# gavrissh/training-operator

Hardware: AMD Instinct MI355X
Metric: job×node fit evals/sec + gang placements/sec, 1M-node inventory, 1/2/4/8 GPUs (higher is better)
Workload: dtype int64

## Files before the change

training-operator_amd/csrc/pe_kernels.h:

```cpp
#pragma once
#include <hip/hip_runtime.h>
#include <stdint.h>

namespace pe {

constexpr int D = 4;
constexpr uint64_t SCORE_MAX = (1ull << 40) - 1;
constexpr uint64_t NO_KEY = ~0ull;
constexpr int64_t NEVER = INT64_MIN;

struct alignas(64) ReqRec {
  int64_t q[D];
  uint32_t need;
  uint32_t pad_[7];
};
static_assert(sizeof(ReqRec) == 64, "ReqRec must be 64 B");

struct alignas(32) ReqRec32 {
  int32_t q[D];
  uint32_t need;
  uint32_t pad_[3];
};
static_assert(sizeof(ReqRec32) == 32, "ReqRec32 must be 32 B");

struct CandHdr {
  int32_t n;
  int32_t flags;
  uint64_t limit;
};
static_assert(sizeof(CandHdr) == 16, "CandHdr must be 16 B");
constexpr int32_t CAND_TIMEOUT = -1;
constexpr int32_t CAND_CORRUPT = -2;

__host__ __device__ inline size_t cand_group_bytes(int K) { return sizeof(CandHdr) + (size_t)K * sizeof(uint64_t); }

constexpr int FM_CH = 4;
constexpr int FM_JT = 256;
constexpr int SC_M = 16;
constexpr int SC_GT = 4;
constexpr int SC_SPAN = 64 * SC_M;
constexpr int SC_WPB = 16;
constexpr int MG_CAP = 16384;
constexpr int MG_THREADS = 1024;
constexpr int MG_SEL = 1024;

constexpr int AGG_SEG_JOBS = 256;
constexpr int64_t AGG_SEG_BYTES = 48 * 1024;
struct AggSegHdr {
  int64_t j0;
  int32_t nj, ng, nc;
  int32_t g0, c0;
  int32_t narrow;
};
static_assert(sizeof(AggSegHdr) == 32, "AggSegHdr must be 32 B");
__host__ __device__ inline int64_t agg_r16(int64_t x) { return (x + 15) & ~int64_t(15); }
struct AggKeys {
  int nd = 4;
  int fb = 1;
};
constexpr int AGG_MAX_KEYS = 16;
__host__ __device__ inline int64_t agg_req_bytes(int64_t nc, int nd, bool narrow) {
  return narrow ? 16 + agg_r16(nc * 4 * nd) : nc * 8 * nd;
}
__host__ __device__ inline void agg_seg_layout(int64_t nj, int64_t ng, int64_t nc, bool v1, int64_t off[7],
                                               AggKeys ak = AggKeys{}, bool narrow = false) {
  off[0] = (int64_t)sizeof(AggSegHdr);
  off[1] = off[0] + agg_r16((nj + 1) * 4);
  off[2] = off[1] + (v1 ? agg_r16(nj * 4) : 0);
  off[3] = off[2] + agg_r16(ng * 4);
  off[4] = off[3] + agg_r16((ng + 1) * 4);
  off[5] = off[4] + agg_req_bytes(nc, ak.nd, narrow);
  off[6] = off[5] + agg_r16(nc * ak.fb);
}
__host__ __device__ inline void agg_out_layout(int64_t J, int64_t off[4], AggKeys ak = AggKeys{}) {
  off[0] = 0;
  off[1] = agg_r16(J * 8 * ak.nd);
  off[2] = off[1] + agg_r16(J * 4);
  off[3] = off[2] + agg_r16(J * (ak.fb == 1 ? 1 : 2));
}

hipError_t launch_pg_agg_segments(hipStream_t s, int mode, const uint8_t* blob, const int64_t* seg_off, int64_t nseg,
                                  int64_t nbytes0, uint8_t* out, int64_t J, uint32_t* flag, uint32_t flag_val,
                                  uint32_t* done_ctr, AggKeys ak = AggKeys{});
constexpr int64_t AGG_KARG_BYTES = 512;
struct AggKarg {
  alignas(16) uint8_t b[AGG_KARG_BYTES];
};
hipError_t launch_pg_agg_karg(hipStream_t s, int mode, const AggKarg& blob, int64_t nbytes, uint8_t* out, int64_t J,
                              uint32_t* flag, uint32_t flag_val, AggKeys ak = AggKeys{});
hipError_t launch_pg_min_resources(hipStream_t s, int mode, int64_t n_jobs, const int32_t* job_group_off,
                                   const int32_t* min_member, const int32_t* group_replicas,
                                   const int32_t* group_cont_off, const int64_t* cont_req,
                                   const uint8_t* cont_flags, int64_t* out_res, uint8_t* out_present,
                                   int32_t* out_members, uint8_t* out_overflow);
hipError_t launch_pg_agg_wide(hipStream_t s, int mode, int64_t n_jobs, int n_keys, const int32_t* job_group_off,
                              const int32_t* min_member, const int32_t* group_replicas,
                              const int32_t* group_cont_off, const uint64_t* req_lo, const uint64_t* req_hi,
                              const uint32_t* cont_flags, uint64_t* out_lo, int64_t* out_hi, uint8_t* out_flag);

__host__ __device__ inline int64_t fm_word_index(int64_t j, int64_t c, int64_t Wt) {
  return ((j >> 4) * Wt + (c >> 2)) * 64 + (j & 15) * 4 + (c & 3);
}
hipError_t launch_fit_mask(hipStream_t s, const int64_t* res, int64_t stride, const uint32_t* labels,
                           int64_t Ns, int64_t Wt, const ReqRec* jobs, int64_t J, int64_t tiles_per_wave,
                           uint64_t* mask, unsigned long long* counts);

hipError_t launch_compress_res(hipStream_t s, const int64_t* res, int32_t* res32, int64_t stride, int64_t Ns,
                               const int* shift);
hipError_t launch_fit_mask32(hipStream_t s, const int32_t* res32, int64_t stride, const uint32_t* labels,
                             int64_t Ns, int64_t Wt, const ReqRec32* jobs, int64_t J, int64_t tiles_per_wave,
                             uint64_t* mask, unsigned long long* counts);

constexpr int CODE_FIELDS = 5;
constexpr int CODE_MAXV = 128;
struct CodeSpec {
  int off[CODE_FIELDS];
  int width[CODE_FIELDS];
  int nvals[CODE_FIELDS];
  uint32_t guard;
  int therm;
};
constexpr int FC_CH = 16;
constexpr int FC_JT = 64;

hipError_t launch_encode_nodes(hipStream_t s, const int64_t* res, int64_t stride, const uint32_t* labels, int64_t Ns,
                               int64_t n_pad, CodeSpec spec, const int64_t* vals, const uint32_t* needs, uint32_t* X);
hipError_t launch_fit_mask_coded(hipStream_t s, int therm, const uint32_t* X, int64_t Ns, int64_t node_stride,
                                 const uint32_t* jcode, uint32_t not_guard, int64_t J, int64_t tiles_per_wave,
                                 uint64_t* mask, unsigned long long* counts);

constexpr int PL_MAX = 32;
constexpr int PL_R = 4;
constexpr int PL_BLK = 64 * PL_R * 32;
struct PlaneSpec {
  int32_t n;
  int32_t kind[PL_MAX];
  int64_t val[PL_MAX];
};
hipError_t launch_encode_planes(hipStream_t s, const int64_t* res, int64_t stride, const uint32_t* labels,
                                int64_t Ns, int64_t nblk, const PlaneSpec& spec, const PlaneSpec* spec_d,
                                uint32_t* planes, unsigned long long* zero = nullptr,
                                int64_t n_zero = 0);
hipError_t launch_fit_mask_planes(hipStream_t s, const uint32_t* planes, int64_t nblk, const uint64_t* jcode,
                                  int64_t J, int64_t jobs_per_wave, uint32_t* mask, unsigned long long* counts);
hipError_t launch_fit_mask_planes_rows(hipStream_t s, const uint32_t* planes, int64_t nblk, const uint64_t* jcode,
                                       int64_t J, int64_t R, uint32_t* mask, unsigned long long* counts,
                                       int64_t pitch_blk, unsigned long long* unit_ctr = nullptr);
hipError_t launch_encode_planes_sets(hipStream_t s, const int64_t* res, int64_t stride, const uint32_t* labels,
                                     int64_t Ns, int64_t nblk, const PlaneSpec* specs, int nsets, uint32_t* planes);
hipError_t launch_fit_mask_planes_sets(hipStream_t s, const uint32_t* planes, int64_t nblk, const uint64_t* jcode,
                                       const int64_t* meta, int nsets, int64_t R, uint32_t* mask,
                                       unsigned long long* counts, int64_t pitch_blk);

constexpr int LD_MAXF = 4;
constexpr int LD_MAXL = 4;
constexpr int LD_MAXNEED = 64;
constexpr int LD_CODE = 16;
constexpr int LD_NEED_SLOT = 15;
__host__ __device__ constexpr int lds_field_off(int fi, int n4, int n3, int n2) {
  return fi <= n4                ? 4 * fi
         : fi <= n4 + n3         ? 4 * n4 + 3 * (fi - n4)
         : fi <= n4 + n3 + n2    ? 4 * n4 + 3 * n3 + 2 * (fi - n4 - n3)
                                 : 4 * n4 + 3 * n3 + 2 * n2 + (fi - n4 - n3 - n2);
}
__host__ __device__ constexpr int lds_need_slot(int n4, int n3, int n2, int n1) {
  return 4 * n4 + 3 * n3 + 2 * n2 + n1;
}
constexpr int LD_THREADS = 1024;
struct LdsSpec {
  int32_t nf;
  int32_t dim[LD_MAXF];
  int32_t L[LD_MAXF];
  uint32_t div[LD_MAXF][LD_MAXL];
  uint32_t mod[LD_MAXF][LD_MAXL];
  int32_t pbase[LD_MAXF][LD_MAXL];
  int32_t vlo[LD_MAXF][LD_MAXL];
  int32_t nv[LD_MAXF][LD_MAXL];
  int32_t nneed, need_pbase, nplanes, nfold;
  int32_t nx, xprod;
  int32_t xstride[LD_MAXF];
  uint32_t needs[LD_MAXNEED];
  int32_t fold_dim[D];
  int64_t fold_val[D];
  int64_t voff[LD_MAXF];
  int64_t m[LD_MAXF];
};
hipError_t launch_node_ranks(hipStream_t s, const int64_t* res, int64_t stride, const uint32_t* labels, int64_t Ns,
                             int64_t npad, const LdsSpec* spec, const int64_t* vals, uint32_t* ranks, uint32_t* aux);
hipError_t launch_fit_mask_lds(hipStream_t s, int W, const int shape[4], const LdsSpec* spec, int nplanes,
                               const uint32_t* ranks, int64_t npad, const uint32_t* aux, int64_t nblk,
                               const uint16_t* codes, int64_t J, int64_t R, int64_t Tpad, int64_t pitch_bytes,
                               uint8_t* mask, uint32_t* slots, uint32_t* units = nullptr);
hipError_t launch_lds_counts(hipStream_t s, const uint32_t* slots, const uint32_t* rows, int64_t nslots,
                             unsigned long long* counts);

hipError_t launch_prep_nodes(hipStream_t s, const int64_t* res, int64_t stride, int64_t Ns, uint64_t id_base,
                             uint64_t* kn, uint32_t* lo );
hipError_t launch_scan(hipStream_t s, const int64_t* res, int64_t stride, const uint32_t* labels, const uint64_t* kn,
                       const uint32_t* lo, int64_t Ns, uint64_t id_base, const ReqRec* groups, int Wg, uint64_t* cand,
                       int32_t* cnt, uint64_t* bound, int nwaves);

hipError_t launch_merge(hipStream_t s, const uint64_t* cand, const int32_t* cnt, const uint64_t* bound,
                        int nwaves, int K, uint8_t* out, int Wg);

constexpr int WK_ROUND = 1024;
constexpr int WK_MAXR = 16384;
constexpr uint64_t WK_INVALID = ~0ull;
#ifndef WK_MULTI
#define WK_MULTI 2
#endif
#ifndef WK_MULTI_AFTER
#define WK_MULTI_AFTER 1
#endif
struct WalkIndex {
  uint64_t* sk;
  int64_t* sr;
  uint32_t* sl;
  uint32_t* pos;
  uint64_t* rmin;
  int64_t* rmax;
  uint32_t* ror;
  int32_t* ovl;
  int32_t* ovl_n;
  uint32_t* in_ovl;
  uint32_t* ovl_idx;
  int64_t* ovl_res;
  uint32_t* ovl_lab;
  uint64_t* ovl_kn;
  unsigned long long* stat;
  int64_t sstride, nr;
};
hipError_t launch_walk_prep(hipStream_t s, const int64_t* res, int64_t stride, int64_t Ns, const uint64_t* kn,
                            const uint32_t* labels, uint64_t* kin, const WalkIndex& w, uint32_t* slow = nullptr);
hipError_t launch_walk_switch(hipStream_t s, const int64_t* res, int64_t stride, const uint32_t* labels, int64_t Ns,
                              const uint32_t* slow, const WalkIndex& nx);
hipError_t sort_keys_u64(void* temp, size_t* temp_bytes, const uint64_t* in, uint64_t* out, int64_t n, hipStream_t s);
hipError_t launch_walk_build(hipStream_t s, const int64_t* res, int64_t stride, const uint32_t* labels, int64_t Ns,
                             uint64_t id_base, const WalkIndex& w);
hipError_t launch_merge_shards(hipStream_t s, const uint8_t* gath, int world, int Wg, int K, uint8_t* out, uint32_t gen,
                               int64_t rank_stride = 0, const uint64_t* xstatus = nullptr, bool sys_scope = true);
constexpr int XW_THREADS = 256;
hipError_t launch_xwait(hipStream_t s, const uint8_t* gath, int world, int Wg, int K, int64_t rank_stride,
                        uint32_t in_gen, int64_t timeout_ticks, uint64_t* xstatus);
constexpr int RM_THREADS = 256, RM_MAX_WORLD = 16;
constexpr size_t RM_MAX_LDS = 64 * 1024;
size_t merge_ranked_lds(int world, int K);
hipError_t launch_merge_ranked(hipStream_t s, const uint8_t* gath, int world, int Wg, int K, uint8_t* out, uint32_t gen,
                               int64_t rank_stride = 0, const uint64_t* xstatus = nullptr, bool sys_scope = true);
hipError_t launch_empty_groups(hipStream_t s, int Wg, int K, uint8_t* out, uint32_t gen);
hipError_t launch_stall(hipStream_t s, int64_t ticks);
hipError_t launch_walk(hipStream_t s, const ReqRec* groups, int Wg, int K, const WalkIndex& w, const int64_t* res,
                       int64_t stride, const uint32_t* labels, int64_t Ns, uint64_t id_base, uint8_t* out,
                       uint32_t gen = 0, int K_stride = 0);

hipError_t launch_apply(hipStream_t s, int64_t* res, int64_t stride, const int64_t* upd, int64_t n, uint64_t id_base,
                        uint64_t* kn, uint32_t* lo, const uint32_t* labels, const WalkIndex* w,
                        const WalkIndex* nx = nullptr);

struct NodeUpd {
  int64_t local;
  int64_t res[D];
  uint32_t labels;
  int32_t island;
};
static_assert(sizeof(NodeUpd) == 48, "NodeUpd must be 48 B");
hipError_t launch_scatter_nodes(hipStream_t s, int64_t* res, int64_t* res0, int64_t stride, uint32_t* labels,
                                int32_t* island, const NodeUpd* upd, int64_t n);

constexpr int CP_THREADS = 256;
constexpr int CP_NPT = 4;
constexpr int CP_SPAN = CP_THREADS * CP_NPT;
constexpr int CP_TS = 64;
constexpr uint64_t CP_CAP_MAX = 2147483647;
__host__ __device__ inline int64_t cap_node_blocks(int64_t Ns) { return (Ns + CP_SPAN - 1) / CP_SPAN; }
struct alignas(32) CapShape {
  int64_t q[D];
  uint64_t m[D];
  uint32_t sh[D];
  uint32_t need;
  uint32_t pad_[3];
};
static_assert(sizeof(CapShape) == 96, "CapShape must be 96 B");
struct CapAcc {
  uint64_t slots;
  uint32_t max_node;
  uint32_t nodes;
};
static_assert(sizeof(CapAcc) == 16, "CapAcc must be 16 B");
hipError_t launch_gang_capacity(hipStream_t s, const int64_t* res, int64_t stride, const uint32_t* labels, int64_t Ns,
                                const CapShape* shapes, int64_t S, CapAcc* partials, CapAcc* out);

constexpr int DM_MAX_DOMAINS = 65536;
struct DomPick {
  uint32_t shape;
  int32_t count;
};
struct DomSel {
  uint64_t slots;
  int32_t domain;
  uint32_t feasible;
};
static_assert(sizeof(DomPick) == 8 && sizeof(DomSel) == 16, "DomPick / DomSel layout");
hipError_t launch_gang_capacity_domains(hipStream_t s, const int64_t* res, int64_t stride, const uint32_t* labels,
                                        const int32_t* island, int64_t Ns, const CapShape* shapes, int64_t S,
                                        int n_domains, uint64_t* dom_slots, uint32_t* dom_nodes);
hipError_t launch_domain_select(hipStream_t s, const uint64_t* dom_slots, int64_t s0, int64_t S, int n_domains,
                                const DomPick* picks, int64_t P, DomSel* out);

constexpr int TR_MAX_LEVELS = 4;
struct TreePick {
  uint32_t shape;
  int32_t count;
  int32_t max_level;
  int32_t pad_;
};
struct TreeSel {
  uint64_t slots;
  int32_t domain;
  int32_t level;
};
static_assert(sizeof(TreePick) == 16 && sizeof(TreeSel) == 16, "TreePick / TreeSel layout");
struct TreeLevels {
  int32_t n_levels;
  int32_t size[TR_MAX_LEVELS];
  int32_t col[TR_MAX_LEVELS];
  int32_t pitch;
};
hipError_t launch_tree_rollup(hipStream_t s, const uint64_t* lo_slots, const uint32_t* lo_nodes, int64_t lo_pitch,
                              const int32_t* start, const int32_t* child, int n_parents, int width, int64_t S,
                              uint64_t* up_slots, uint32_t* up_nodes, int64_t up_pitch);
hipError_t launch_tree_select(hipStream_t s, const uint64_t* leaf_slots, const uint64_t* upper_slots, int64_t s0,
                              int64_t S, const TreeLevels& levels, const TreePick* picks, int64_t P, TreeSel* out,
                              uint32_t* feasible);

}
```

training-operator_amd/csrc/pe_kernels.hip:

```cpp
#include <type_traits>

#include "pe_kernels.h"
#include "pe_wave.h"

namespace pe {

__device__ __forceinline__ uint64_t umin64(uint64_t a, uint64_t b) { return a < b ? a : b; }

__device__ __forceinline__ uint64_t wave_min_u64(uint64_t v) {
#pragma unroll
  for (int off = 32; off >= 1; off >>= 1) v = umin64(v, __shfl_xor(v, off, 64));
  return v;
}


__device__ __forceinline__ bool add_ovf(int64_t a, int64_t b, int64_t* r) { return __builtin_add_overflow(a, b, r); }
__device__ __forceinline__ bool mul_ovf(int64_t a, int64_t b, int64_t* r) { return __builtin_mul_overflow(a, b, r); }

template <int ND>
struct AggJob {
  int64_t acc[ND];
  uint32_t pres, members;
  int32_t pod_cnt;
  bool ovf;
// ... 1912 lines not shown
  if (tid < world) cnt[tid] = lds_lower_bound(lk + tid * K, hn[tid], L);
  __syncthreads();
  const int c = (K + 1 + world - 1) / world;
  int T = 0, have = 0;
  uint64_t U = 0;
  for (int r = 0; r < world; ++r) {
    const int hd = min(cnt[r], c);
    T += cnt[r];
    have += hd;
    if (hd > 0) U = umax64(U, lk[r * K + hd - 1]);
  }
  if (tid < world)
    mc[tid] = have >= K + 1 ? lds_lower_bound(lk + tid * K, cnt[tid], U + 1) : cnt[tid];
  __syncthreads();
  int M = 0, mx = 0, mq[RM_MAX_WORLD];
#pragma unroll
  for (int q = 0; q < RM_MAX_WORLD; ++q) {
    mq[q] = q < world ? mc[q] : 0;
    M += mq[q];
    mx = max(mx, mq[q]);
  }
  int top = 1;
  while (top * 2 <= mx) top *= 2;
  uint64_t* ok = lk + (size_t)world * K;
  for (int t = tid; t < M; t += RM_THREADS) {
    int r = 0, idx = t;
    while (idx >= mc[r]) {
      idx -= mc[r];
      ++r;
    }
    const uint64_t k = lk[r * K + idx];
    int pos[RM_MAX_WORLD];
#pragma unroll
    for (int q = 0; q < RM_MAX_WORLD; ++q) pos[q] = 0;
    for (int st = top; st > 0; st >>= 1) {
#pragma unroll
      for (int q = 0; q < RM_MAX_WORLD; ++q) {
        const int p = pos[q] + st;
        if (q < world && q != r && p <= mq[q] && lk[q * K + p - 1] < k) pos[q] = p;
      }
    }
    int rank = idx;
#pragma unroll
    for (int q = 0; q < RM_MAX_WORLD; ++q) rank += pos[q];
    if (rank <= K) ok[rank] = k;
  }
  __syncthreads();
  const int nout = T < K ? T : K;
  uint64_t* dst = reinterpret_cast<uint64_t*>(og + sizeof(CandHdr));
  for (int i = tid; i < nout; i += RM_THREADS) dst[i] = ok[i];
  if (tid == 0) {
    hp->n = nout;
    hp->limit = T > K ? ok[K] : L;
    if (gen == 0) hp->flags = 0;
  }
  asm volatile("s_waitcnt vmcnt(0)" ::: "memory");
  __syncthreads();
  if (tid == 0 && gen != 0) __hip_atomic_store(&hp->flags, (int32_t)gen, __ATOMIC_RELEASE, __HIP_MEMORY_SCOPE_SYSTEM);
}

size_t merge_ranked_lds(int world, int K) { return ((size_t)world * K + K + 1) * sizeof(uint64_t); }

hipError_t launch_merge_ranked(hipStream_t s, const uint8_t* gath, int world, int Wg, int K, uint8_t* out, uint32_t gen,
                               int64_t rank_stride, const uint64_t* xstatus, bool sys_scope) {
  if (Wg <= 0) return hipSuccess;
  if (world < 1 || world > RM_MAX_WORLD || K < 1 || merge_ranked_lds(world, K) > RM_MAX_LDS) return hipErrorInvalidValue;
  if (sys_scope)
    hipLaunchKernelGGL(merge_ranked_kernel<true>, dim3(Wg), dim3(RM_THREADS), merge_ranked_lds(world, K), s, gath, world,
                       Wg, K, out, gen, rank_stride, xstatus);
  else
    hipLaunchKernelGGL(merge_ranked_kernel<false>, dim3(Wg), dim3(RM_THREADS), merge_ranked_lds(world, K), s, gath, world,
                       Wg, K, out, gen, rank_stride, xstatus);
  return hipGetLastError();
}

__global__ __launch_bounds__(64) void empty_groups_kernel(int Wg, int K, uint8_t* __restrict__ out, uint32_t gen) {
  write_group(nullptr, 0, 0, NO_KEY, K, blockIdx.x, out, gen);
}

__global__ __launch_bounds__(64) void stall_kernel(int64_t ticks) {
  const long long t0 = wall_clock64();
  while (wall_clock64() - t0 < ticks) __builtin_amdgcn_s_sleep(127);
}

hipError_t launch_stall(hipStream_t s, int64_t ticks) {
  if (ticks <= 0 || ticks > (int64_t)30 * 100000000) return hipErrorInvalidValue;
  hipLaunchKernelGGL(stall_kernel, dim3(1), dim3(64), 0, s, ticks);
  return hipGetLastError();
}

hipError_t launch_empty_groups(hipStream_t s, int Wg, int K, uint8_t* out, uint32_t gen) {
  if (Wg <= 0) return hipSuccess;
  hipLaunchKernelGGL(empty_groups_kernel, dim3(Wg), dim3(64), 0, s, Wg, K, out, gen);
  return hipGetLastError();
}

hipError_t launch_merge(hipStream_t s, const uint64_t* cand, const int32_t* cnt, const uint64_t* bound, int nwaves,
                        int K, uint8_t* out, int Wg) {
  if (Wg <= 0) return hipSuccess;
  hipLaunchKernelGGL(merge_kernel, dim3(Wg), dim3(MG_THREADS), 0, s, cand, cnt, bound, nwaves, K, out);
  return hipGetLastError();
}


__device__ __forceinline__ void overlay_add(const WalkIndex& w, int64_t n, const int64_t (&r)[D], uint32_t lab,
                                            uint64_t Kn) {
  const int32_t i = atomicAdd(w.ovl_n, 1);
  w.ovl[i] = (int32_t)n;
  w.ovl_idx[n] = (uint32_t)i;
#pragma unroll
  for (int d = 0; d < D; ++d) w.ovl_res[d * w.sstride + i] = r[d];
  w.ovl_lab[i] = lab;
  w.ovl_kn[i] = Kn;
}

__global__ __launch_bounds__(256) void walk_prep_kernel(const int64_t* __restrict__ res, int64_t stride, int64_t Ns,
                                                        const uint64_t* __restrict__ kn,
                                                        const uint32_t* __restrict__ labels, uint64_t* __restrict__ kin,
                                                        WalkIndex w, uint32_t* __restrict__ slow) {
  const int64_t n = (int64_t)blockIdx.x * blockDim.x + threadIdx.x;
  if (n >= Ns) return;
  const int64_t r[D] = {res[n], res[stride + n], res[2 * stride + n], res[3 * stride + n]};
  const bool neg = (r[0] | r[1] | r[2] | r[3]) < 0;
  const uint64_t K = kn[n];
  uint64_t k = K;
  if (neg) {
    k = WK_INVALID;
  } else if (K == KEY_SLOW) {
    k = WK_INVALID;
    if (slow) {
      slow[n] = 1u;
    } else {
      w.in_ovl[n] = 1u;
      overlay_add(w, n, r, labels[n], KEY_SLOW);
    }
  }
  kin[n] = k;
}

hipError_t launch_walk_prep(hipStream_t s, const int64_t* res, int64_t stride, int64_t Ns, const uint64_t* kn,
                            const uint32_t* labels, uint64_t* kin, const WalkIndex& w, uint32_t* slow) {
  if (Ns <= 0) return hipSuccess;
  hipLaunchKernelGGL(walk_prep_kernel, dim3((unsigned)((Ns + 255) / 256)), dim3(256), 0, s, res, stride, Ns, kn, labels,
                     kin, w, slow);
  return hipGetLastError();
}

__global__ __launch_bounds__(256) void walk_switch_kernel(const int64_t* __restrict__ res, int64_t stride,
                                                          const uint32_t* __restrict__ labels, int64_t Ns,
                                                          const uint32_t* __restrict__ slow, WalkIndex nx) {
  const int64_t n = (int64_t)blockIdx.x * blockDim.x + threadIdx.x;
  if (n >= Ns) return;
  if (nx.in_ovl[n]) {
    const uint32_t p = nx.pos[n];
    if (p != ~0u) {
      nx.sk[p] = WK_INVALID;
      nx.pos[n] = ~0u;
    }
  } else if (slow[n]) {
    const int64_t r[D] = {res[n], res[stride + n], res[2 * stride + n], res[3 * stride + n]};
    nx.in_ovl[n] = 1u;
    overlay_add(nx, n, r, labels[n], KEY_SLOW);
  }
}

hipError_t launch_walk_switch(hipStream_t s, const int64_t* res, int64_t stride, const uint32_t* labels, int64_t Ns,
                              const uint32_t* slow, const WalkIndex& nx) {
  if (Ns <= 0) return hipSuccess;
  hipLaunchKernelGGL(walk_switch_kernel, dim3((unsigned)((Ns + 255) / 256)), dim3(256), 0, s, res, stride, labels, Ns,
                     slow, nx);
  return hipGetLastError();
}

__global__ __launch_bounds__(WK_ROUND) void walk_build_kernel(const int64_t* __restrict__ res, int64_t stride,
                                                              const uint32_t* __restrict__ labels, int64_t Ns,
                                                              uint64_t id_base, WalkIndex w) {
  __shared__ int64_t mx[D][WK_ROUND / 64];
  __shared__ uint32_t orl[WK_ROUND / 64];
  const int tid = threadIdx.x, lane = tid & 63, wave = tid >> 6;
  const int64_t r = blockIdx.x;
  const int64_t i = r * WK_ROUND + tid;
  const uint64_t K = i < Ns ? w.sk[i] : WK_INVALID;
  int64_t v[D] = {INT64_MIN, INT64_MIN, INT64_MIN, INT64_MIN};
  uint32_t lab = 0;
  if (K != WK_INVALID) {
    const int64_t n = (int64_t)((K & 0xFFFFFFull) - id_base);
    w.pos[n] = (uint32_t)i;
#pragma unroll
    for (int d = 0; d < D; ++d) {
      v[d] = res[d * stride + n];
      w.sr[d * w.sstride + i] = v[d];
    }
    lab = labels[n];
    w.sl[i] = lab;
  }
#pragma unroll
  for (int d = 0; d < D; ++d)
    for (int off = 32; off >= 1; off >>= 1) {
      const int64_t o = __shfl_xor(v[d], off, 64);
      v[d] = o > v[d] ? o : v[d];
    }
  for (int off = 32; off >= 1; off >>= 1) lab |= __shfl_xor(lab, off, 64);
  if (lane == 0) {
#pragma unroll
    for (int d = 0; d < D; ++d) mx[d][wave] = v[d];
    orl[wave] = lab;
  }
  __syncthreads();
  if (tid < D) {
    int64_t m = INT64_MIN;
    for (int k = 0; k < WK_ROUND / 64; ++k) m = mx[tid][k] > m ? mx[tid][k] : m;
    w.rmax[tid * w.nr + r] = m;
  } else if (tid == D) {
    uint32_t o = 0;
    for (int k = 0; k < WK_ROUND / 64; ++k) o |= orl[k];
    w.ror[r] = o;
    w.rmin[r] = w.sk[r * WK_ROUND];
  }
}

hipError_t launch_walk_build(hipStream_t s, const int64_t* res, int64_t stride, const uint32_t* labels, int64_t Ns,
                             uint64_t id_base, const WalkIndex& w) {
  if (Ns <= 0) return hipSuccess;
  hipLaunchKernelGGL(walk_build_kernel, dim3((unsigned)w.nr), dim3(WK_ROUND), 0, s, res, stride, labels, Ns, id_base,
                     w);
  return hipGetLastError();
}

__device__ __forceinline__ void step_append(TopkShared& s, int T0, int* cnt, uint64_t k, bool take) {
  const uint64_t bal = __ballot(take);
  if (bal == 0) return;
  const int rank = __builtin_amdgcn_mbcnt_hi((uint32_t)(bal >> 32), __builtin_amdgcn_mbcnt_lo((uint32_t)bal, 0));
  int base = 0;
  if (take && rank == 0) base = atomicAdd(cnt, __popcll(bal));
  base = T0 + __shfl(base, __ffsll((unsigned long long)bal) - 1, 64);
  if (take && base + rank < MG_CAP) s.keys[base + rank] = k;
}

#ifdef PE_WALK_PROF
__device__ unsigned long long walk_prof[32];
#define WPT(i) unsigned long long wpt##i = wall_clock64()
#else
#define WPT(i)
#endif

__global__ __launch_bounds__(WK_ROUND) void walk_kernel(const ReqRec* __restrict__ groups, int K, int Kst, WalkIndex w,
                                                        const int64_t* __restrict__ res, int64_t stride,
                                                        const uint32_t* __restrict__ labels, int64_t Ns,
                                                        uint64_t id_base, uint8_t* __restrict__ out, uint32_t gen) {
  static_assert(WK_ROUND == MG_THREADS, "the walk uses the merge's block-wide selection");
  __shared__ TopkShared s;
  __shared__ uint32_t cbits[WK_MAXR / 32];
  __shared__ int start_cnt, below[2], wcnt[3];
  const int g = blockIdx.x;
  const int tid = threadIdx.x, lane = tid & 63;
  WPT(0);
  const ReqRec rq = groups[g];
  const int64_t q0 = rq.q[0], q1 = rq.q[1], q2 = rq.q[2], q3 = rq.q[3];
  const uint32_t need = rq.need;
  uint64_t sq = (uint64_t)q0 + ((uint64_t)q1 >> 20) + ((uint64_t)q3 >> 24);
  sq = (uint64_t)q0 > SCORE_MAX || (uint64_t)q2 >= (1ull << 20) || sq >= SCORE_MAX ? SCORE_MAX : sq;
  sq = sq < SCORE_MAX ? sq + ((uint64_t)q2 << 20) : sq;
  const bool walk = sq < SCORE_MAX;
  const uint64_t KQ = walk ? sq << 24 : 0;
  const uint64_t KQ2 = !walk ? 0 : sq + 2 >= (1ull << 40) ? ~0ull : (sq + 2) << 24;
  const int64_t nr = w.nr;
  const int nwords = (int)((nr + 31) / 32);
  for (int i = tid; i < nwords; i += WK_ROUND) cbits[i] = 0u;
  if (tid == 0) {
    s.total = 0;
    start_cnt = 0;
    below[0] = below[1] = 0;
    wcnt[0] = wcnt[1] = wcnt[2] = 0;
  }
  __syncthreads();
  if (walk) {
    int cnt = 0;
    for (int64_t r0 = 0; r0 < nr; r0 += WK_ROUND) {
      const int64_t r = r0 + tid;
      bool can = false;
      if (r < nr) {
        cnt += w.rmin[r] < KQ;
        can = q0 <= w.rmax[r] && q1 <= w.rmax[nr + r] && q2 <= w.rmax[2 * nr + r] && q3 <= w.rmax[3 * nr + r] &&
              (w.ror[r] & need) == need;
      }
#ifdef PE_PREPASS_ATOMIC
      if (can) atomicOr(&cbits[r >> 5], 1u << (r & 31));
#else
      const uint64_t bal = __ballot(can);
      const int64_t wr = r0 + (tid & ~63);
      if (lane == 0 && wr < nr) {
        cbits[wr >> 5] = (uint32_t)bal;
        if (wr + 32 < nr) cbits[(wr >> 5) + 1] = (uint32_t)(bal >> 32);
      }
#endif
    }
    for (int off = 32; off >= 1; off >>= 1) cnt += __shfl_xor(cnt, off, 64);
    if (lane == 0 && cnt) atomicAdd(&start_cnt, cnt);
  }
  __syncthreads();
  WPT(1);
  bool done = !walk;
  int rounds = 0;
  int64_t r = walk ? (start_cnt > 0 ? start_cnt - 1 : 0) : nr;
  auto next_round = [&](int64_t from) -> int64_t {
    int64_t wi = from >> 5;
    if (wi >= nwords) return nr;
    uint32_t bits = cbits[wi] & (~0u << (from & 31));
    while (bits == 0) {
      if (++wi >= nwords) return nr;
      bits = cbits[wi];
    }
    return wi * 32 + __ffs(bits) - 1;
  };
  if (!done) r = next_round(r);
  uint64_t xstop = NO_KEY;
  int tests = 0;
  int lo_idx = 0, cnt_certain = 0;
  constexpr int PEND = 4;
  int pend_n = 0;
  int pend_end[PEND];
  uint64_t pend_b[PEND];
  auto pend_push = [&](int end, uint64_t b) {
    if (pend_n == PEND) {
#pragma unroll
      for (int i = 0; i + 1 < PEND; ++i) {
        pend_end[i] = pend_end[i + 1];
        pend_b[i] = pend_b[i + 1];
      }
      --pend_n;
    }
#pragma unroll
    for (int i = 0; i < PEND; ++i)
      if (i == pend_n) {
        pend_end[i] = end;
        pend_b[i] = b;
      }
    ++pend_n;
  };
  int Tcur = 0;
  int step = 0;
  auto compact = [&]() {
    const int T2 = Tcur < MG_CAP ? Tcur : MG_CAP;
    const uint64_t* sk = topk_sort(s, T2, K);
    const int m = T2 < K + 1 ? T2 : K + 1;
    uint64_t v = tid < m ? sk[tid] : 0;
    __syncthreads();
    if (tid < m) s.keys[tid] = v;
    __syncthreads();
    Tcur = m;
    return m;
  };
  auto step_begin = [&]() -> int* {
    if (tid == 0) wcnt[(step + 1) % 3] = 0;
    return &wcnt[step % 3];
  };
  auto step_end = [&]() {
    Tcur += wcnt[step % 3];
    ++step;
  };
  uint64_t rm_r = !done && r < nr ? w.rmin[r] : 0;
  while (!done && r < nr) {
    const int T = Tcur < MG_CAP ? Tcur : MG_CAP;
    if (T >= K + 1) {
#ifdef PE_WALK_NO_RM_PREFETCH
      const uint64_t rm = w.rmin[r];
#else
      const uint64_t rm = rm_r;
#endif
      const uint64_t X = rm > KQ2 ? rm - KQ2 : 0;
      while (pend_n > 0 && pend_b[0] < X) {
        cnt_certain += pend_end[0] - lo_idx;
        lo_idx = pend_end[0];
#pragma unroll
        for (int i = 0; i + 1 < PEND; ++i) {
          pend_end[i] = pend_end[i + 1];
          pend_b[i] = pend_b[i + 1];
        }
        --pend_n;
      }
#ifdef PE_WALK_CHECK
      if (cnt_certain >= K + 1) {
        __shared__ int full2;
        if (tid == 0) full2 = 0;
        __syncthreads();
        int cf = 0;
        for (int i = tid; i < T; i += WK_ROUND) cf += s.keys[i] < X;
        for (int off = 32; off >= 1; off >>= 1) cf += __shfl_xor(cf, off, 64);
        if (lane == 0 && cf) atomicAdd(&full2, cf);
        __syncthreads();
        if (tid == 0 && full2 < cnt_certain)
          printf("walk check: g %d early full %d < certain %d (lo_idx %d T %d X %llx)\n", g, full2, cnt_certain, lo_idx, T,
                 (unsigned long long)X);
        __syncthreads();
      }
#endif
      if (cnt_certain >= K + 1) {
        xstop = X;
        break;
      }
      int c = 0;
      for (int i = lo_idx + tid; i < T; i += WK_ROUND) c += s.keys[i] < X;
      for (int off = 32; off >= 1; off >>= 1) c += __shfl_xor(c, off, 64);
      if (lane == 0 && c) atomicAdd(&below[tests & 1], c);
      __syncthreads();
      const int nb = below[tests & 1];
      if (tid == 0) below[(tests + 1) & 1] = 0;
      ++tests;
#ifdef PE_WALK_CHECK
      {
        __shared__ int full;
        if (tid == 0) full = 0;
        __syncthreads();
        int cf = 0;
        for (int i = tid; i < T; i += WK_ROUND) cf += s.keys[i] < X;
        for (int off = 32; off >= 1; off >>= 1) cf += __shfl_xor(cf, off, 64);
        if (lane == 0 && cf) atomicAdd(&full, cf);
        __syncthreads();
        if (tid == 0 && full != cnt_certain + nb)
          printf("walk check: g %d full %d != certain %d + %d (lo_idx %d T %d pend %d X %llx)\n", g, full, cnt_certain,
                 nb, lo_idx, T, pend_n, (unsigned long long)X);
        __syncthreads();
      }
#endif
      if (cnt_certain + nb >= K + 1) {
        xstop = X;
        break;
      }
    }
    int64_t rr[WK_MULTI];
    int nstep = 1;
    rr[0] = r;
    if (rounds >= WK_MULTI_AFTER)
      for (; nstep < WK_MULTI; ++nstep) {
        const int64_t nx = next_round(rr[nstep - 1] + 1);
        if (nx >= nr) break;
        rr[nstep] = nx;
      }
    const int64_t r_next = next_round(rr[nstep - 1] + 1);
    const uint64_t rm_next = r_next < nr ? w.rmin[r_next] : 0;
    uint64_t k[WK_MULTI];
#pragma unroll
    for (int u = 0; u < WK_MULTI; ++u) {
      k[u] = NO_KEY;
      const int64_t i = rr[u < nstep ? u : 0] * WK_ROUND + tid;
      if (u < nstep && i < Ns) {
#ifdef PE_WALK_COND_LOAD
        const uint64_t Kn = w.sk[i];
        if (Kn != WK_INVALID)
          k[u] = node_key(w.sr[i], w.sr[w.sstride + i], w.sr[2 * w.sstride + i], w.sr[3 * w.sstride + i], w.sl[i], q0,
                          q1, q2, q3, need, Kn & 0xFFFFFFull);
#else
        const uint64_t Kn = w.sk[i];
        const int64_t s0 = w.sr[i], s1 = w.sr[w.sstride + i], s2 = w.sr[2 * w.sstride + i], s3 = w.sr[3 * w.sstride + i];
        const uint32_t sl = w.sl[i];
        const uint64_t kk = node_key(s0, s1, s2, s3, sl, q0, q1, q2, q3, need, Kn & 0xFFFFFFull);
        k[u] = Kn != WK_INVALID ? kk : NO_KEY;
#endif
      }
    }
    int* const cnt = step_begin();
#pragma unroll
    for (int u = 0; u < WK_MULTI; ++u)
      if (u < nstep) step_append(s, Tcur, cnt, k[u], k[u] != NO_KEY);
    __syncthreads();
    step_end();
    pend_push(Tcur, r_next < nr ? (rm_next > KQ ? rm_next - KQ : 0) : NO_KEY);
    if (Tcur > MG_CAP - WK_MULTI * WK_ROUND) {
      const int m = compact();
      lo_idx = cnt_certain = pend_n = 0;
      pend_push(m, m > 0 ? s.keys[m - 1] : 0);
    }
    r = r_next;
    rm_r = rm_next;
    rounds += nstep;
  }
  WPT(2);
#ifndef WK_OV
#define WK_OV 8
#endif
  constexpr int OV = WK_OV;
  const int no = *w.ovl_n;
  const uint64_t klim = xstop > NO_KEY - KQ2 ? NO_KEY : xstop + KQ2;
  for (int i0 = 0; i0 < no; i0 += OV * WK_ROUND) {
    uint64_t kn[OV];
#pragma unroll
    for (int u = 0; u < OV; ++u) {
      const int i = i0 + u * WK_ROUND + tid;
      kn[u] = i < no ? w.ovl_kn[i] : 0;
    }
    uint64_t k[OV];
#pragma unroll
    for (int u = 0; u < OV; ++u) {
      const int i = i0 + u * WK_ROUND + tid;
      k[u] = NO_KEY;
      if (i < no && (kn[u] == KEY_SLOW || (kn[u] >= KQ && kn[u] < klim)))
        k[u] = node_key(w.ovl_res[i], w.ovl_res[w.sstride + i], w.ovl_res[2 * w.sstride + i],
                        w.ovl_res[3 * w.sstride + i], w.ovl_lab[i], q0, q1, q2, q3, need, id_base + (uint64_t)w.ovl[i]);
    }
    if (Tcur > MG_CAP - OV * WK_ROUND) compact();
    int* const cnt = step_begin();
#pragma unroll
    for (int u = 0; u < OV; ++u) step_append(s, Tcur, cnt, k[u], k[u] < xstop);
    __syncthreads();
    step_end();
  }
  __syncthreads();
  WPT(3);
  const int T = Tcur < MG_CAP ? Tcur : MG_CAP;
  const uint64_t* sk = topk_sort(s, T, K, xstop);
  WPT(4);
  write_group(sk, T < K ? T : K, 0, T > K ? sk[K] : NO_KEY, Kst, g, out, gen);
  if (tid == 0 && w.stat) {
    atomicAdd(&w.stat[0], (unsigned long long)rounds);
    atomicAdd(&w.stat[1], (unsigned long long)no);
  }
#ifdef PE_WALK_PROF
  __syncthreads();
  WPT(5);
  if (tid == 0) {
    atomicAdd(&walk_prof[0], wpt1 - wpt0);
    atomicAdd(&walk_prof[1], wpt2 - wpt1);
    atomicAdd(&walk_prof[2], wpt3 - wpt2);
    atomicAdd(&walk_prof[3], wpt4 - wpt3);
    atomicAdd(&walk_prof[4], wpt5 - wpt4);
    atomicAdd(&walk_prof[5], 1ull);
    atomicAdd(&walk_prof[6], (unsigned long long)no);
    atomicAdd(&walk_prof[7], (unsigned long long)rounds);
    atomicAdd(&walk_prof[8], (unsigned long long)T);
    atomicMax(&walk_prof[9], wpt5 - wpt0);
    atomicMax(&walk_prof[10], wpt2 - wpt1);
    atomicMax(&walk_prof[11], wpt3 - wpt2);
    atomicMax(&walk_prof[12], wpt4 - wpt3);
    atomicMax(&walk_prof[13], (unsigned long long)rounds);
    atomicMax(&walk_prof[14], (unsigned long long)T);
    atomicMax(&walk_prof[15], wpt1 - wpt0);
    if (wpt5 - wpt0 > 3500) {
      atomicAdd(&walk_prof[16], 1ull);
      atomicAdd(&walk_prof[17], wpt1 - wpt0);
      atomicAdd(&walk_prof[18], wpt2 - wpt1);
      atomicAdd(&walk_prof[19], wpt3 - wpt2);
      atomicAdd(&walk_prof[20], wpt4 - wpt3);
      atomicAdd(&walk_prof[21], wpt5 - wpt4);
      atomicAdd(&walk_prof[22], (unsigned long long)rounds);
      atomicAdd(&walk_prof[23], (unsigned long long)T);
      atomicAdd(&walk_prof[24], (unsigned long long)no);
      atomicAdd(&walk_prof[25], (unsigned long long)tests);
    }
  }
#endif
}

hipError_t launch_walk(hipStream_t s, const ReqRec* groups, int Wg, int K, const WalkIndex& w, const int64_t* res,
                       int64_t stride, const uint32_t* labels, int64_t Ns, uint64_t id_base, uint8_t* out,
                       uint32_t gen, int K_stride) {
  if (Wg <= 0) return hipSuccess;
  const int Kst = K_stride > 0 ? K_stride : K;
  if (w.nr > WK_MAXR || K + 1 > WK_ROUND || K > Kst) return hipErrorInvalidValue;
  hipLaunchKernelGGL(walk_kernel, dim3((unsigned)Wg), dim3(WK_ROUND), 0, s, groups, K, Kst, w, res, stride, labels, Ns,
                     id_base, out, gen);
#ifdef PE_WALK_PROF
  static int launches = 0;
  if (++launches % 500 == 0) {
    unsigned long long p[32];
    (void)hipStreamSynchronize(s);
    (void)hipMemcpyFromSymbol(p, HIP_SYMBOL(walk_prof), sizeof(p));
    const double n = (double)p[5], us = 100.0;
    fprintf(stderr, "walk prof over %.0f blocks (us/block): setup+prepass %.2f walk %.2f overlay %.2f sort %.2f write %.2f"
                    " | overlay %.0f rounds %.2f T %.0f\n", n, p[0] / n / us, p[1] / n / us, p[2] / n / us,
            p[3] / n / us, p[4] / n / us, p[6] / n, p[7] / n, p[8] / n);
    fprintf(stderr, "walk prof max: block %.2f us setup %.2f walk %.2f overlay %.2f sort %.2f | rounds %llu T %llu\n",
            p[9] / us, p[15] / us, p[10] / us, p[11] / us, p[12] / us, p[13], p[14]);
    const double ns = (double)(p[16] ? p[16] : 1);
    fprintf(stderr, "walk prof slow blocks (> 35 us): %.0f (%.2f%%): setup %.2f walk %.2f overlay %.2f sort %.2f write %.2f"
                    " us | rounds %.2f T %.0f overlay %.0f tests %.2f\n", (double)p[16], 100.0 * p[16] / n, p[17] / ns / us,
            p[18] / ns / us, p[19] / ns / us, p[20] / ns / us, p[21] / ns / us, p[22] / ns, p[23] / ns, p[24] / ns, p[25] / ns);
    unsigned long long t[8];
    (void)hipMemcpyFromSymbol(t, HIP_SYMBOL(topk_prof), sizeof(t));
    const double c = (double)t[0];
    fprintf(stderr, "topk_sort: %.0f calls, T %.0f, C %.0f, bitonic %.0f, hist+select %.2f us, rank %.2f us per call\n",
            c, t[1] / c, t[3] / c, (double)t[2], t[4] / c / us, t[5] / c / us);
  }
#endif
  return hipGetLastError();
}


__global__ __launch_bounds__(256) void apply_kernel(int64_t* __restrict__ res, int64_t stride,
                                                    const int64_t* __restrict__ upd, int64_t n, uint64_t id_base,
                                                    uint64_t* __restrict__ kn, uint32_t* __restrict__ lo,
                                                    const uint32_t* __restrict__ labels, WalkIndex w, int walk,
                                                    WalkIndex nx, int pend) {
  const int64_t i = (int64_t)blockIdx.x * blockDim.x + threadIdx.x;
  if (i >= n) return;
  const int64_t* u = upd + i * (D + 1);
  const int64_t node = u[0];
#pragma unroll
  for (int d = 0; d < D; ++d) res[d * stride + node] = u[1 + d];
  uint64_t K;
  uint32_t l1, l3;
  node_prep(u[1], u[2], u[3], u[4], id_base + (uint64_t)node, K, l1, l3);
  if (kn) {
    kn[node] = K;
    lo[node] = l1;
    lo[stride + node] = l3;
  }
  if (walk) {
    const uint32_t p = w.pos[node];
    if (p != ~0u) {
      w.sk[p] = WK_INVALID;
      w.pos[node] = ~0u;
    }
    const int64_t r[D] = {u[1], u[2], u[3], u[4]};
    if (atomicExch(&w.in_ovl[node], 1u) == 0u) {
      overlay_add(w, node, r, labels[node], K);
    } else {
      const uint32_t i = w.ovl_idx[node];
#pragma unroll
      for (int d = 0; d < D; ++d) w.ovl_res[d * w.sstride + i] = r[d];
      w.ovl_kn[i] = K;
    }
    if (pend) {
      if (atomicExch(&nx.in_ovl[node], 1u) == 0u) {
        overlay_add(nx, node, r, labels[node], K);
      } else {
        const uint32_t i = nx.ovl_idx[node];
#pragma unroll
        for (int d = 0; d < D; ++d) nx.ovl_res[d * nx.sstride + i] = r[d];
        nx.ovl_kn[i] = K;
      }
    }
  }
}

hipError_t launch_apply(hipStream_t s, int64_t* res, int64_t stride, const int64_t* upd, int64_t n, uint64_t id_base,
                        uint64_t* kn, uint32_t* lo, const uint32_t* labels, const WalkIndex* w,
                        const WalkIndex* nx) {
  if (n <= 0) return hipSuccess;
  const WalkIndex none{};
  hipLaunchKernelGGL(apply_kernel, dim3((unsigned)((n + 255) / 256)), dim3(256), 0, s, res, stride, upd, n, id_base,
                     kn, lo, labels, w ? *w : none, w ? 1 : 0, (w && nx) ? *nx : none, (w && nx) ? 1 : 0);
  return hipGetLastError();
}


__global__ __launch_bounds__(256) void scatter_nodes_kernel(int64_t* __restrict__ res, int64_t* __restrict__ res0,
                                                            int64_t stride, uint32_t* __restrict__ labels,
                                                            int32_t* __restrict__ island,
                                                            const NodeUpd* __restrict__ upd, int64_t n) {
  const int64_t i = (int64_t)blockIdx.x * blockDim.x + threadIdx.x;
  if (i >= n) return;
  const NodeUpd u = upd[i];
#pragma unroll
  for (int d = 0; d < D; ++d) {
    res[d * stride + u.local] = u.res[d];
    res0[d * stride + u.local] = u.res[d];
  }
  labels[u.local] = u.labels;
  island[u.local] = u.island;
}

hipError_t launch_scatter_nodes(hipStream_t s, int64_t* res, int64_t* res0, int64_t stride, uint32_t* labels,
                                int32_t* island, const NodeUpd* upd, int64_t n) {
  if (n <= 0) return hipSuccess;
  hipLaunchKernelGGL(scatter_nodes_kernel, dim3((unsigned)((n + 255) / 256)), dim3(256), 0, s, res, res0, stride,
                     labels, island, upd, n);
  return hipGetLastError();
}

}
```

Measured before the change: 46180 billion.

## Adapt walk step width to candidate yield and batch loads per width

```diff
diff --git a/training-operator_amd/csrc/pe_kernels.h b/training-operator_amd/csrc/pe_kernels.h
--- a/training-operator_amd/csrc/pe_kernels.h
+++ b/training-operator_amd/csrc/pe_kernels.h
@@ -208,9 +208,6 @@
 constexpr uint64_t WK_INVALID = ~0ull;
 #ifndef WK_MULTI
 #define WK_MULTI 2
-#endif
-#ifndef WK_MULTI_AFTER
-#define WK_MULTI_AFTER 1
 #endif
 struct WalkIndex {
   uint64_t* sk;
diff --git a/training-operator_amd/csrc/pe_kernels.hip b/training-operator_amd/csrc/pe_kernels.hip
--- a/training-operator_amd/csrc/pe_kernels.hip
+++ b/training-operator_amd/csrc/pe_kernels.hip
@@ -2238,6 +2238,7 @@
   WPT(1);
   bool done = !walk;
   int rounds = 0;
+  int want = 1;
   int64_t r = walk ? (start_cnt > 0 ? start_cnt - 1 : 0) : nr;
   auto next_round = [&](int64_t from) -> int64_t {
     int64_t wi = from >> 5;
@@ -2366,34 +2367,55 @@
     }
     int64_t rr[WK_MULTI];
     int nstep = 1;
+    int64_t last = r;
     rr[0] = r;
-    if (rounds >= WK_MULTI_AFTER)
-      for (; nstep < WK_MULTI; ++nstep) {
-        const int64_t nx = next_round(rr[nstep - 1] + 1);
-        if (nx >= nr) break;
-        rr[nstep] = nx;
-      }
-    const int64_t r_next = next_round(rr[nstep - 1] + 1);
+#pragma unroll
+    for (int u = 1; u < WK_MULTI; ++u) {
+      rr[u] = r;
+      if (nstep == u && u < want) {
+        const int64_t nx = next_round(last + 1);
+        if (nx < nr) {
+          rr[u] = last = nx;
+          nstep = u + 1;
+        }
+      }
+    }
+    const int64_t r_next = next_round(last + 1);
     const uint64_t rm_next = r_next < nr ? w.rmin[r_next] : 0;
     uint64_t k[WK_MULTI];
-#pragma unroll
-    for (int u = 0; u < WK_MULTI; ++u) {
-      k[u] = NO_KEY;
-      const int64_t i = rr[u < nstep ? u : 0] * WK_ROUND + tid;
-      if (u < nstep && i < Ns) {
-#ifdef PE_WALK_COND_LOAD
-        const uint64_t Kn = w.sk[i];
-        if (Kn != WK_INVALID)
-          k[u] = node_key(w.sr[i], w.sr[w.sstride + i], w.sr[2 * w.sstride + i], w.sr[3 * w.sstride + i], w.sl[i], q0,
-                          q1, q2, q3, need, Kn & 0xFFFFFFull);
-#else
-        const uint64_t Kn = w.sk[i];
-        const int64_t s0 = w.sr[i], s1 = w.sr[w.sstride + i], s2 = w.sr[2 * w.sstride + i], s3 = w.sr[3 * w.sstride + i];
-        const uint32_t sl = w.sl[i];
-        const uint64_t kk = node_key(s0, s1, s2, s3, sl, q0, q1, q2, q3, need, Kn & 0xFFFFFFull);
-        k[u] = Kn != WK_INVALID ? kk : NO_KEY;
-#endif
-      }
+    auto step_keys = [&](auto width) {
+      constexpr int N = decltype(width)::value;
+      uint64_t Kn[N];
+      int64_t s0[N], s1[N], s2[N], s3[N];
+      uint32_t sl[N];
+      bool in[N];
+#pragma unroll
+      for (int u = 0; u < N; ++u) {
+        const int64_t i0 = rr[u] * WK_ROUND + tid;
+        in[u] = i0 < Ns;
+        const int64_t i = in[u] ? i0 : Ns - 1;
+        Kn[u] = w.sk[i];
+        s0[u] = w.sr[i];
+        s1[u] = w.sr[w.sstride + i];
+        s2[u] = w.sr[2 * w.sstride + i];
+        s3[u] = w.sr[3 * w.sstride + i];
+        sl[u] = w.sl[i];
+      }
+      __builtin_amdgcn_sched_barrier(0);
+#pragma unroll
+      for (int u = 0; u < WK_MULTI; ++u) k[u] = NO_KEY;
+#pragma unroll
+      for (int u = 0; u < N; ++u) {
+        const uint64_t kk = node_key(s0[u], s1[u], s2[u], s3[u], sl[u], q0, q1, q2, q3, need, Kn[u] & 0xFFFFFFull);
+        k[u] = in[u] && Kn[u] != WK_INVALID ? kk : NO_KEY;
+      }
+    };
+    static_assert(WK_MULTI >= 1 && WK_MULTI <= 4, "one straight-line copy of the step per width");
+    switch (nstep) {
+      case 1: step_keys(std::integral_constant<int, 1>{}); break;
+      case 2: step_keys(std::integral_constant<int, WK_MULTI >= 2 ? 2 : 1>{}); break;
+      case 3: step_keys(std::integral_constant<int, WK_MULTI >= 3 ? 3 : 1>{}); break;
+      default: step_keys(std::integral_constant<int, WK_MULTI>{}); break;
     }
     int* const cnt = step_begin();
 #pragma unroll
@@ -2410,6 +2432,11 @@
     r = r_next;
     rm_r = rm_next;
     rounds += nstep;
+    static_assert((WK_MULTI + 1) * WK_ROUND <= MG_CAP - WK_MULTI * WK_ROUND, "a wide step must not reach the compaction");
+    const int missing = K + 1 - Tcur;
+    want = 1;
+#pragma unroll
+    for (int n = 1; n < WK_MULTI; ++n) want += missing > 0 && n * Tcur < missing * rounds;
   }
   WPT(2);
 #ifndef WK_OV
```

Result: no change. 46200 billion (median of 4 runs) (+0.0%).
